# fan1994song/Sentinel

Hardware: AMD Instinct MI355X
Metric: flow-check decisions/sec (node) + % HBM roofline, 10M resources, 1/2/4/8 GPU (higher is better)
Workload: dtype int64; 1 GPU; config3: 10M resources Zipf(1.1), 60% QPS / 10% THREAD / 15% WarmUp / 15% RateLimiter, acquireCount 1 (90%) or 2-5, RT~Exp(20ms) exits; events_per_batch_per_gpu=134217728, entries_per_batch_per_gpu=122837294, parallelism=resource-sharded x1, trace=config-3 batch, seed 3

## Files before the change

### sentinel_amd/csrc/sf_engine.cpp

```cpp
#include <functional>

#include "sf_host.h"

static thread_local std::string g_err;

int fail(int code, const std::string& msg) {
    g_err = msg;
    return code;
}

extern "C" {

int sf_abi_version(void) { return SF_ABI_VERSION; }
const char* sf_last_error(void) { return g_err.c_str(); }

void sf_config_default(sf_config* c) {
    std::memset(c, 0, sizeof *c);
    c->sample_count = 2; c->interval_ms = 1000; c->occupy_timeout_ms = 500; c->cold_factor = 3;
    c->statistic_max_rt = 5000; c->max_resources = 1024; c->max_batch = 1u << 20;
    c->param_capacity = 1u << 16; c->shard_count = 1; c->shard_index = 0; c->device = 0;
    c->cluster_sample_count = 10; c->cluster_interval_ms = 1000; c->exceed_count = 1.0;
    c->max_occupy_ratio = 1.0; c->max_flow_ids = 1024; c->aux_capacity = 65536;
}

static int slot_create(Slot& sl) {
    for (auto& x : sl.evs) HIP_TRY(hipEventCreate(&x));
    for (hipEvent_t* x : {&sl.sorted, &sl.done, &sl.end, &sl.core})
        HIP_TRY(hipEventCreateWithFlags(x, hipEventDisableTiming));
    return SF_OK;
}

void sf_destroy(sf_engine* e) {
    if (!e) return;
    for (hipStream_t x : {e->sstream, e->stream, e->h2d, e->d2h}) if (x) hipStreamSynchronize(x);
    for (Slot& sl : e->slot) { sl.wpool.clear(); sl.pkpool.clear(); }
    for (DevPool* p : {&e->pool, &e->user_dev, &e->user_host, &e->tok.tw.pool, &e->rls.ws.pool, &e->cc.ws.pool, &e->dg.ws.pool, &e->rep.ml_pool})
        p->clear();
    if (e->comm) ncclCommDestroy(e->comm);
    for (Slot& sl : e->slot) {
        const PkStage& p = sl.pk;
        for (hipEvent_t x : {p.h2d, p.d2h, p.consumed, sl.sorted, sl.done, sl.end, sl.core}) if (x) hipEventDestroy(x);
        for (hipEvent_t x : sl.evs) if (x) hipEventDestroy(x);
    }
    for (auto& x : e->rep.ml_ev) if (x) hipEventDestroy(x);
    if (e->ev_en) hipEventDestroy(e->ev_en);
    for (hipStream_t x : {e->h2d, e->d2h, e->stream, e->stream2, e->stream3, e->stream4, e->sstream}) if (x) hipStreamDestroy(x);
    if (e->enstream && e->en_own) hipStreamDestroy(e->enstream);
    delete e;
}

static int work_fill(sf_engine* e, Work& w, DevPool& m) {
    const sf_config& c = e->cfg;
    const size_t N = c.max_batch, R = e->R;
    SF_TRY(m.alloc(&w.keys_in, nz(N * 4))); SF_TRY(m.alloc(&w.keys_out, nz(N * 4))); SF_TRY(m.alloc(&w.perm, nz(N * 4)));
    SF_TRY(m.alloc(&w.pv_in, nz(N * sizeof(PackedEvO)))); SF_TRY(m.alloc(&w.pv_out, nz(N * sizeof(PackedEvO))));
    SF_TRY(m.alloc(&w.err, nz(4)));
    SF_TRY(m.alloc(&w.head_scan, nz(N * 4)));
    SF_TRY(m.alloc(&w.seg_start, nz((N + 1) * 4))); SF_TRY(m.alloc(&w.seg_res, nz(N * 4))); SF_TRY(m.alloc(&w.n_seg, nz(4)));
    SF_TRY(m.alloc(&w.s_meta, nz(N * 4)));
    SF_TRY(m.alloc(&w.s_eref, nz(N * 8))); SF_TRY(m.alloc(&w.s_cts, nz(N * 8)));
    SF_TRY(m.alloc(&w.s_nargs, nz(N))); SF_TRY(m.alloc(&w.s_atag, nz(N * SF_MAX_ARGS))); SF_TRY(m.alloc(&w.s_abits, nz(N * SF_MAX_ARGS * 8)));
    SF_TRY(m.alloc(&w.v_status, nz(N))); SF_TRY(m.alloc(&w.v_wait, nz(N * 4))); SF_TRY(m.alloc(&w.v_rule, nz(N * 2)));
    {
        hipError_t he = query_temp_bytes((uint32_t)N, &w.sort_tmp_bytes, &w.scan_tmp_bytes, &w.pscan_tmp_bytes);
        if (he != hipSuccess) return fail(SF_ERR_DEVICE, "scan temp size query");
    }
    SF_TRY(m.alloc(&w.sort_tmp, nz(w.sort_tmp_bytes)));
    SF_TRY(m.alloc(&w.scan_tmp, nz(w.scan_tmp_bytes)));
    SF_TRY(m.alloc(&w.pscan_tmp, nz(w.pscan_tmp_bytes)));
    w.heavy_min = c.heavy_min_events ? c.heavy_min_events : 512;
    {
        int dev = 0, ncu = 0;
        if (hipGetDevice(&dev) != hipSuccess ||
            hipDeviceGetAttribute(&ncu, hipDeviceAttributeMultiprocessorCount, dev) != hipSuccess) ncu = 256;
        w.stream_grid = 2u * (uint32_t)(ncu > 0 ? ncu : 256);
        w.fill_grid = 8u * (uint32_t)(ncu > 0 ? ncu : 256);
    }
    const size_t SC = std::min<size_t>(N, R) + 1;
    w.seg_cap = (uint32_t)SC;
    SF_TRY(m.alloc(&w.segflag, nz(SC * 4))); SF_TRY(m.alloc(&w.seg_mode, nz(SC))); SF_TRY(m.alloc(&w.lcounts, nz(2 * LCLS * 4)));
    {
        size_t off = 0;
        for (int k = 0; k < LCLS; k++) {
            const size_t lo_len = k == 0 ? 1 : (k == 1 ? 2 : ((size_t)1 << (k - 1)) + 1);
            const size_t cap = lo_len > w.heavy_min ? 0 : std::min<size_t>(SC, N / lo_len + 1);
            w.loff[k] = (uint32_t)off;
            w.lcap[k] = (uint32_t)cap;
            off += cap;
        }
        SF_TRY(m.alloc(&w.light_list, nz(off * 4)));
// ... 6 lines not shown
    SF_TRY(m.alloc(&w.acc_hw, nz((size_t)w.acc_cap * ACC_BYTES))); SF_TRY(m.alloc(&w.acc_sec, nz((size_t)w.acc_cap * ACC_BYTES)));
    SF_TRY(m.alloc(&w.acc_hw_base, nz(SC * 4))); SF_TRY(m.alloc(&w.acc_sec_base, nz(SC * 4))); SF_TRY(m.alloc(&w.seg_hw0, nz(SC * 8)));
    SF_TRY(m.alloc(&w.seg_sec0, nz(SC * 8))); SF_TRY(m.alloc(&w.seg_nhw, nz(SC * 4))); SF_TRY(m.alloc(&w.seg_nsec, nz(SC * 4)));
    SF_TRY(m.alloc(&w.hticks, nz((N / (w.heavy_min + 1) + 2) * 8)));
    SF_TRY(m.alloc(&w.sticks, nz((N / (w.heavy_min + 1) + 2) * 8)));
    SF_TRY(m.alloc(&w.stream_list, nz(SC * 4)));
    SF_TRY(m.alloc(&w.xw_list, nz((N / XW_MIN + 1) * 4)));
    SF_TRY(m.alloc(&w.passbits, nz((N / 64 + 2) * 8)));
    SF_TRY(m.alloc(&w.exit_of, nz(N * 4)));
    SF_TRY(m.alloc(&w.lxfar, nz((N / 64 + 2) * 8)));
    SF_TRY(m.alloc(&w.thr_rec, nz(N * 8)));
    SF_TRY(m.alloc(&w.tile_rc, nz((size_t)w.fill_tile_cap * 4))); SF_TRY(m.alloc(&w.seg_rb, nz(SC * 4))); SF_TRY(m.alloc(&w.seg_re, nz(SC * 4)));
    SF_TRY(m.alloc(&w.vs_cursor, nz(VS_CURSORS(N) * 4)));
    SF_TRY(m.alloc(&w.s_origin, nz(N * 4))); SF_TRY(m.alloc(&w.s_oslot, nz(N * 4))); SF_TRY(m.alloc(&w.ox_cnt, nz(8 * 4)));
    SF_TRY(m.alloc(&w.ox_bflags, nz((N / OX_TILE + 1) * 4))); SF_TRY(m.alloc(&w.ox_bseg, nz((N / OX_TILE + 1) * 8)));
    return SF_OK;
}

static int alloc_work(sf_engine* e, Slot& sl) {
    const int rc = work_fill(e, sl.w, sl.wpool);
    if (rc) { sl.wpool.clear(); sl.w = Work{}; sl.aflags = nullptr; return rc; }
    sl.ready = true;
    return SF_OK;
}

static int create(sf_engine* e);
int sf_create(const sf_config* cfg, sf_engine** out) {
    if (!cfg || !out) return fail(SF_ERR_INVALID, "null argument");
    *out = nullptr;
    const sf_config& c = *cfg;
    if (c.sample_count <= 0 || c.sample_count > SF_MAX_SAMPLE_COUNT || c.interval_ms <= 0 ||
        c.interval_ms % c.sample_count != 0)
        return fail(SF_ERR_INVALID, "sample_count/interval_ms invalid (LeapArray.java:70-87)");
    if (c.max_resources == 0 || c.max_batch == 0) return fail(SF_ERR_INVALID, "max_resources/max_batch must be > 0");
    if (c.shard_count == 0 || c.shard_index >= c.shard_count) return fail(SF_ERR_INVALID, "bad shard");
    int ndev = 0;
    if (hipGetDeviceCount(&ndev) != hipSuccess || ndev <= 0)
        return fail(SF_ERR_DEVICE, "no HIP device visible: the engine has no CPU fallback");
    if (c.device < 0 || c.device >= ndev) return fail(SF_ERR_DEVICE, "device ordinal out of range");
    HIP_TRY(hipSetDevice(c.device));
    hipDeviceProp_t prop;
    HIP_TRY(hipGetDeviceProperties(&prop, c.device));
    if (std::strncmp(prop.gcnArchName, "gfx950", 6) != 0)
        return fail(SF_ERR_DEVICE, std::string("engine is built for gfx950, device is ") + prop.gcnArchName);

    sf_engine* e = new sf_engine();
// ... 63 lines not shown
    HIP_TRY(hipMemsetAsync(st.ptab, 0, pcap * sizeof(ParamSlot), e->stream));
    SF_TRY(e->pool.alloc(&st.pins, nz(256 * 16 * sizeof(unsigned int))));
    SF_TRY(e->pool.alloc(&st.xw_stats, nz(4 * sizeof(unsigned long long))));
    HIP_TRY(hipMemset(e->st.xw_stats, 0, 4 * sizeof(unsigned long long)));
    HIP_TRY(hipMemsetAsync(st.pins, 0, 256 * 16 * sizeof(unsigned int), e->stream));
    HIP_TRY(hipMemsetAsync(st.err, 0, sizeof(int32_t), e->stream));
    HIP_TRY(launch_init_state(st, e->stream));
    e->tok.ts.err = st.err;
    e->tok.ts.exceed_count = c.exceed_count;
    e->tok.ts.shard_count = c.shard_count; e->tok.ts.shard_index = c.shard_index;
    e->tok.ts.max_occupy_ratio = c.max_occupy_ratio;
    SF_TRY(e->pool.alloc(&e->tok.d_sum, nz(sizeof(int64_t))));
    SF_TRY(e->pool.alloc(&st.last_fetch, nz(R * sizeof(int64_t))));
    SF_TRY(e->pool.alloc(&st.last_ts, nz(sizeof(int64_t))));
    {
        const int64_t t_min = INT64_MIN;
        HIP_TRY(hipMemcpyAsync(st.last_ts, &t_min, 8, hipMemcpyHostToDevice, e->stream));
    }
    HIP_TRY(hipMemsetAsync(st.last_fetch, 0xff, R * sizeof(int64_t), e->stream));
    SF_TRY(e->pool.alloc(&e->en, nz(sizeof(EntryNode))));
    SF_TRY(e->pool.alloc(&e->en_acc, nz(sizeof(EntryAcc))));
    HIP_TRY(launch_entry_init(e->en, st.max_rt, e->stream));

    SF_TRY(alloc_work(e, e->slot[0]));
    HIP_TRY(hipStreamSynchronize(e->stream));
    return SF_OK;
}

extern "C++" int local_of(const sf_engine* e, uint32_t res, uint32_t* l) {
    if (res % e->cfg.shard_count != e->cfg.shard_index) return 0;
    *l = res / e->cfg.shard_count;
    return *l < e->R;
}

static void acc_timing(sf_engine* e, Slot& sl) {
    if (!sl.timed) return;
    sl.timed = false;
    hipEvent_t* ev = sl.evs;
    float a = 0, b2 = 0, c = 0, d = 0;
    hipEventElapsedTime(&a, ev[0], ev[1]);
    hipEventElapsedTime(&b2, ev[1], ev[2]);
    hipEventElapsedTime(&c, ev[2], ev[3]);
    hipEventElapsedTime(&d, ev[3], ev[4]);
    float cl = 0, li = 0, hd = 0, hf = 0, hs = 0;
    hipEventElapsedTime(&cl, ev[10], ev[2]);
    hipEventElapsedTime(&li, ev[5], ev[9]);
    if (e->st.n_window_rules) {
        float lq = 0;
        hipEventElapsedTime(&lq, ev[5], ev[16]);
        li = std::max(li, lq);
    }
    hipEventElapsedTime(&hd, ev[5], ev[7]);
    hipEventElapsedTime(&hf, ev[7], ev[8]);
    hipEventElapsedTime(&hs, ev[11], ev[12]);
    e->stats.classify_ms += cl; e->stats.light_ms += li;
    e->stats.heavy_decide_ms += hd; e->stats.heavy_fill_ms += hf; e->stats.stream_ms += hs;
    e->stats.sort_ms += a + b2;
    e->stats.decide_ms += c;
    e->stats.scatter_ms += d;
    e->stats.total_ms += a + b2 + c + d;
}

static int batch_error(int err) {
// ... 578 lines not shown
    e->stats.n_launches++;
}

static int finish_sync(sf_engine* e, Slot& sl, const StagePlan& vout, uint32_t n, bool plain) {
    hipStream_t s = e->stream;
    HIP_TRY(hipEventRecord(sl.core, s));
    HIP_TRY(hipEventRecord(sl.done, s));
    HIP_TRY(hipEventRecord(sl.end, s));
    slot_enqueued(e, sl, n);
    sl.timed = plain && e->timing;
    SF_TRY(vout.download(d2h_on(s)));
    int32_t err = 0;
    uint32_t nseg = 0;
    HIP_TRY(hipMemcpyAsync(&err, sl.w.err, 4, hipMemcpyDeviceToHost, s));
    if (plain) HIP_TRY(hipMemcpyAsync(&nseg, sl.w.n_seg, 4, hipMemcpyDeviceToHost, s));
    HIP_TRY(hipStreamSynchronize(s));
    if (plain) {
        e->stats.n_segments = nseg;
        acc_timing(e, sl);
    }
    return batch_error(err);
}

static int decide_view(sf_engine* e, Slot& sl, DevState& stl, const DevBatch& b, const DevVerdicts& dv,
                       uint32_t p, uint32_t q, bool with_ox, DevBatch& v, DevVerdicts& dvv) {
    hipStream_t s = e->stream;
    Work& w = sl.w;
    v = b;
    v.n = q - p; v.base = p;
    v.res = b.res + p; v.ts = b.ts + p; v.cnt = b.cnt + p; v.flags = b.flags + p;
    v.eref = b.eref ? b.eref + p : nullptr; v.cts = b.cts ? b.cts + p : nullptr;
    v.nargs = b.nargs ? b.nargs + p : nullptr;
    v.atag = b.atag ? b.atag + p : nullptr; v.abits = b.abits ? b.abits + p : nullptr;
    v.origin = b.origin ? b.origin + p : nullptr; v.ctx = b.ctx ? b.ctx + p : nullptr;
    v.sys = e->sys_mask + p; v.vprev = dv.status + p;
    dvv = DevVerdicts{dv.status + p, dv.wait ? dv.wait + p : nullptr, dv.rule ? dv.rule + p : nullptr};
    hipError_t le = launch_sort(stl, w, v, e->cfg.shard_count, e->cfg.shard_index, e->key_bits, s, sl.evs, false);
    OxPlan plan{};
    if (le == hipSuccess && with_ox) {
        SF_TRY(prepare_origins(e, sl, v, s, &plan));
        stl.xtab = e->st.xtab; stl.xcap_mask = e->st.xcap_mask; stl.ax_cap = e->st.ax_cap;
    }
    if (le == hipSuccess)
        le = launch_decide(stl, w, v, dvv, s, e->serial ? s : e->stream2, e->serial ? s : e->stream3,
                           e->serial ? s : e->stream4, sl.evs, false, with_ox ? &plan : nullptr);
    if (le == hipSuccess && with_ox) w.ox_dirty = false;
    if (le != hipSuccess) return fail(SF_ERR_DEVICE, std::string("launch: ") + hipGetErrorString(le));
    return SF_OK;
}

using PreSort = std::function<hipError_t(hipStream_t, int32_t*)>;
struct PackedHook { PreSort pre; bool acsr; uint32_t n_arg_events; };

static int submit_sys_rounds(sf_engine* e, Slot& sl, const DevBatch& staged, const DevVerdicts& dv, const StagePlan& vout,
                             bool with_ox, const PreSort* pre) {
    DevBatch b = staged;
    const uint32_t n = b.n;
    hipStream_t s = e->stream, ss = e->serial ? e->stream : e->sstream;
    Work& w = sl.w;
    SF_TRY(sys_buffers_ensure(e));
// ... 25 lines not shown
        SF_TRY(decide_view(e, sl, stl, b, dv, p, q, with_ox, v, dvv));
        if (qi[1]) le = sys_plan_fix(stl, b, dv, e->sys_mask, e->sys, p, q, e->sys_plan, e->sys_pa, e->sys_pb, s);
        if (le == hipSuccess) le = launch_entry_node(stl, v, dvv.status, e->en, e->en_acc, s);
        if (le != hipSuccess) return fail(SF_ERR_DEVICE, std::string("launch: ") + hipGetErrorString(le));
        p = q;
        rounds++;
    }
    e->stats.sys_rounds += rounds;
    return finish_sync(e, sl, vout, n, false);
}

static int submit_core(sf_engine* e, const sf_event_batch* in, sf_verdicts* out, bool async,
                       const uint8_t* forced = nullptr, const PackedHook* hook = nullptr) {
    if (!e || !in || !out || !out->status) return fail(SF_ERR_INVALID, "null argument");
    if (in->n == 0) return SF_OK;
    SF_TRY(check_event_batch(e, in));
    if (e->sys.check && e->cfg.shard_count > 1 && !forced)
        return fail(SF_ERR_UNSUPPORTED, "SystemRules on a sharded engine: use sf_system_plan + sf_submit_forced "
                                        "+ sf_entry_node_add (the node-wide round protocol)");
    const uint32_t n = in->n;
    hipStream_t s = e->stream, ss = e->serial ? e->stream : e->sstream;
    const bool with_ox = in->origin || e->st.xmap;
    async = async && in->mem != SF_MEM_HOST && out->mem != SF_MEM_HOST && !e->sys.check && !forced;
    if (!async || (with_ox && !e->st.xtab)) SF_TRY(drain(e));
    SF_TRY(reserve_for_batch(e, in, with_ox, hook ? hook->n_arg_events : in->n));
    const PreSort* pre = hook ? &hook->pre : nullptr;
    for (Slot& x : e->slot) {
        if (!async || x.ready) continue;
        HIP_TRY(hipStreamSynchronize(s));
        SF_TRY(alloc_work(e, x));
    }
    Slot& sl = e->slot[e->cur];
    SF_TRY(take_slot(e, sl));
    Work& w = sl.w;
    DevBatch b{};
    DevVerdicts dv{};
    StagePlan vout(false, out->mem == SF_MEM_HOST);
    SF_TRY(stage_batch(e, in, out, ss, b, dv, vout));
    b.acsr = hook && hook->acsr;
    if (forced) {
        SF_TRY(sys_buffers_ensure(e));
        HIP_TRY(hipMemcpyAsync(e->sys_mask, forced, n, hipMemcpyHostToDevice, ss));
        b.sys = e->sys_mask;
    }
    if (e->sys.check && !forced) return submit_sys_rounds(e, sl, b, dv, vout, with_ox, pre);
    if (sl.used) HIP_TRY(hipStreamWaitEvent(ss, e->auth.of && b.origin ? sl.end : sl.done, 0));
    HIP_TRY(hipMemsetAsync(w.err, 0, sizeof(int32_t), ss));
    if (pre) {
        const hipError_t pe = (*pre)(ss, w.err);
        if (pe != hipSuccess) return fail(SF_ERR_DEVICE, std::string("pre-sort: ") + hipGetErrorString(pe));
    }
    SF_TRY(auth_apply(e, sl, b, ss));
    DevState stl = e->st;
    stl.err = w.err;
    hipError_t le = launch_sort(stl, w, b, e->cfg.shard_count, e->cfg.shard_index, e->key_bits, ss, sl.evs, e->timing);
    if (le != hipSuccess) return fail(SF_ERR_DEVICE, std::string("launch: ") + hipGetErrorString(le));
    OxPlan plan{};
    if (with_ox) {
        SF_TRY(prepare_origins(e, sl, b, ss, &plan));
        stl.xtab = e->st.xtab; stl.xcap_mask = e->st.xcap_mask; stl.ax_cap = e->st.ax_cap;
    }
    HIP_TRY(hipEventRecord(sl.sorted, ss));
    HIP_TRY(hipStreamWaitEvent(s, sl.sorted, 0));
    const bool side = async && !e->serial && e->side_mode != 0;
    le = launch_decide(stl, w, b, dv, s, e->serial ? s : e->stream2, e->serial ? s : e->stream3,
                       e->serial ? s : e->stream4, sl.evs, e->timing,
                       with_ox ? &plan : nullptr, false, side ? e->enstream : nullptr);
    if (le != hipSuccess) return fail(SF_ERR_DEVICE, std::string("launch: ") + hipGetErrorString(le));
    if (with_ox) w.ox_dirty = false;
    if (!side && !forced) {
        SF_TRY(en_fence(e));
        le = launch_entry_node(stl, b, dv.status, e->en, e->en_acc, s);
        if (le != hipSuccess) return fail(SF_ERR_DEVICE, std::string("entry node: ") + hipGetErrorString(le));
    }
    if (!async) return finish_sync(e, sl, vout, n, true);
    hipStream_t es = side ? e->enstream : s;
    HIP_TRY(hipEventRecord(sl.core, es));
    HIP_TRY(hipEventRecord(sl.done, es));
// ... 931 lines not shown
```

### sentinel_amd/csrc/sf_host.h

```cpp
#pragma once
#include <hip/hip_runtime.h>

#include <algorithm>
#include <cmath>
#include <cstring>
#include <mutex>
#include <string>
#include <vector>

#include "sf_decide.h"
#include "sf_pkargs.h"
#include "sf_xflow.h"
#include "sf_sysx.h"
#include "sf_token.h"
#include "sf_concur.h"
#include "sf_wire.h"
#include "sf_rls.h"
#include "sf_degrade.h"
#include "sf_mem.h"
#include "sf_worksets.h"
#include <rccl/rccl.h>

using namespace sf;

// ... 115 lines not shown
    hipEvent_t h2d = nullptr, d2h = nullptr;
    hipEvent_t consumed = nullptr;
    bool d2h_pending = false, consumed_pending = false;
    const uint8_t* out_status = nullptr;
    int32_t* err_host = nullptr;
    bool sparse = false;
    sf_sparse_verdicts sp{};
    uint32_t* sp_counts = nullptr;
    const unsigned long long* sp_wl = nullptr; const unsigned long long* sp_rl = nullptr;
};

constexpr int SF_SLOTS = 2;
struct Slot {
    Work w{};
    DevPool wpool{HIP_MEM};
    bool ready = false;
    bool used = false;
    bool timed = false;
    hipEvent_t sorted = nullptr;
    hipEvent_t done = nullptr;
    hipEvent_t end = nullptr;
    hipEvent_t core = nullptr;
    hipEvent_t evs[SF_NUM_EVENTS]{};
    PkStage pk;
    DevPool pkpool{HIP_MEM};
    uint8_t* aflags = nullptr;
};

struct sf_engine {
    sf_config cfg{};
    DevPool pool{HIP_MEM};
    DevPool user_dev{HIP_MEM}, user_host{HIP_MEM};
    hipStream_t stream = nullptr, stream2 = nullptr, stream3 = nullptr, stream4 = nullptr;
    hipStream_t sstream = nullptr;
    hipStream_t enstream = nullptr;
    bool en_own = false;
    int side_mode = 3;
    hipEvent_t ev_en = nullptr;
    bool en_async = false;
    bool serial = false;
    uint32_t R = 0, key_bits = 1;
    DevState st{};
    Slot slot[SF_SLOTS];
    int cur = 0, last = 0;
    unsigned pending = 0;
    SysRule sys{};
    SysPlanDev* sys_plan = nullptr; SysExitQ* sys_pa = nullptr; SysEntQ* sys_pb = nullptr;
    uint8_t* sys_ibuf = nullptr;
    uint8_t* sys_mask = nullptr;
    std::vector<uint32_t> flow_pos;
    uint32_t n_flow = 0, n_prule = 0;
    AuthTables auth{};
    uint64_t p_used = 0, p_pending = 0, p_kmax = 0, p_grows = 0;
    GrowBuf stage_in, stage_out;
    StageBuf plan_sb, en_sb;
    bool timing = false;
    sf_stats stats{};
    std::mutex mu;
    TokHost tok;
    CcHost cc;
    RlsHost rls;
    DgHost dg;
    ReportHost rep;
    SxHost sx;
    EntryNode* en = nullptr;
    EntryAcc* en_acc = nullptr;
// ... 15 lines not shown
```

### sentinel_amd/csrc/sf_internal.h

```cpp
#pragma once
#include <hip/hip_runtime.h>
#include <stdint.h>

#include "../../include/sentinel_flow.h"
#include "sf_degrade.h"
#include "sf_authority.h"

namespace sf {

constexpr int64_t WS_NONE = -(1LL << 62);
constexpr int MINUTE = SF_MINUTE_BUCKETS;
constexpr int MAX_RULES = SF_MAX_RULES_PER_RESOURCE;

struct Bucket {
    int64_t ws, pass, block, exc, succ, rt, occ, min_rt;
};
struct Borrow {
    int64_t ws, pass;
};

enum : int32_t { CT_DEFAULT = 0, CT_WARM_UP = 1, CT_RATE_LIMITER = 2, CT_WARM_UP_RATE_LIMITER = 3 };

struct DevRule {
    uint8_t kind, grade;
// ... 109 lines not shown
struct alignas(8) PackedEv { uint32_t idx, meta; };
struct PackedEvO { uint32_t idx, meta, origin; };
constexpr uint32_t PV_DTS_FAR = 0xffffu;

constexpr int LCLS = 16;
#ifndef SF_SHORT_MAX
#define SF_SHORT_MAX 8
#endif
constexpr uint32_t SHORT_MAX = SF_SHORT_MAX;
__host__ __device__ inline int light_class(uint32_t len) {
    if (len <= 1) return 0;
    const int c = 32 - __builtin_clz(len - 1);
    return c < LCLS - 1 ? c : LCLS - 1;
}
#ifndef SF_FILL_TILE
#define SF_FILL_TILE 2048
#endif
constexpr uint32_t FILL_TILE = SF_FILL_TILE;

struct Work {
    uint32_t n;
    uint32_t* keys_in;   uint32_t* keys_out;
    uint32_t* perm;
    PackedEv* pv_in; PackedEv* pv_out;
    int32_t* err;
    bool ox_dirty;
    uint32_t* head;      uint32_t* head_scan;
    uint32_t* seg_start; uint32_t* seg_res; uint32_t* n_seg;
    uint32_t* s_meta;
    int64_t* s_eref; int64_t* s_cts;
    uint8_t* s_nargs; uint8_t* s_atag; uint64_t* s_abits;
    uint8_t* v_status; int32_t* v_wait; uint16_t* v_rule;
    void* sort_tmp; size_t sort_tmp_bytes;
    void* scan_tmp; size_t scan_tmp_bytes;
    uint32_t seg_cap;
    uint32_t* segflag; uint8_t* seg_mode;
    uint32_t* light_list; uint32_t* heavy_list; uint32_t* counters;
    uint32_t* lcounts;
    uint32_t loff[LCLS];
    uint32_t lcap[LCLS];
    int64_t* pcg; void* pscan_tmp; size_t pscan_tmp_bytes;
    void* segs_lb;
    uint2* fill_tiles; uint32_t fill_tile_cap;
    uint32_t* fill_ntiles;
    uint32_t fill_grid;
    void* acc_hw; void* acc_sec; uint32_t acc_cap;
    uint32_t* acc_hw_base; uint32_t* acc_sec_base; int64_t* seg_hw0; int64_t* seg_sec0;
    uint32_t* seg_nhw; uint32_t* seg_nsec;
    uint32_t heavy_min;
    uint32_t stream_grid;
    uint64_t* hticks;
    uint32_t* stream_list;
    uint32_t* xw_list;
    uint64_t* sticks;
    unsigned long long* passbits;
    uint32_t* exit_of;
// ... 5 lines not shown
    uint32_t* s_origin;
    uint32_t* s_oslot;
    uint32_t* ox_cnt;
    uint32_t* ox_bflags;
    uint2* ox_bseg;
    uint4* ox_pairs; uint32_t ox_pairs_cap;
    uint32_t* ox_plist;
    uint32_t* ox_hmap; size_t ox_hmap_n;
    uint32_t* ox_hslot; size_t ox_hslot_n;
    int64_t* ox_thr;
    void* ox_acc; size_t ox_acc_n;
};
constexpr uint32_t OX_TILE = 2048, OX_LIGHT = 512;
enum : int { OXC_HEAVY = 0, OXC_PAIRS = 1, OXC_PLIST = 2, OXC_OVERFLOW = 3, OXC_RESERVED = 4 };
struct OxAcc {
    unsigned long long pass, block, succ, rt, exc, n_touch, min_rt_key;
};
#ifndef SF_VS_REG
#define SF_VS_REG 14
#endif
constexpr uint32_t VS_REG = SF_VS_REG;
inline size_t VS_CURSORS(size_t N) { return 256 + (N >> VS_REG) + 1024 + 16; }

struct DevBatch {
    uint32_t n;
    const uint32_t* res; const int64_t* ts; const int32_t* cnt; const uint8_t* flags;
    const int64_t* eref; const int64_t* cts;
    uint32_t arg_slots; const uint8_t* nargs; const uint8_t* atag; const uint64_t* abits;
    uint32_t arg_stride;
    const uint32_t* aoff; const uint8_t* etag; const uint64_t* ebits;
    uint32_t acsr;
    const uint32_t* origin; const uint32_t* ctx;
    int64_t base;
    const uint8_t* sys;
    const uint8_t* vprev;
    uint8_t marked;
};
struct DevVerdicts { uint8_t* status; int32_t* wait; uint16_t* rule; };

constexpr uint8_t EVF_SYSBLK = 0x80u;
constexpr uint8_t EVF_SYSREASON_SHIFT = 4;
constexpr uint8_t SYS_NONE = 0xFFu;
constexpr uint8_t SYS_INERT = 0xFEu;
constexpr uint8_t SYSR_OTHER = 7;
constexpr uint8_t SYSR_AUTH = 6;
constexpr int64_t EREF_DEAD = -2;

hipError_t query_temp_bytes(uint32_t max_n, size_t* sort_bytes, size_t* scan_bytes, size_t* pscan_bytes);
hipError_t launch_init_state(const DevState& st, hipStream_t s);
hipError_t launch_rdesc(const DevState& st, hipStream_t s);
hipError_t launch_entry_node(const DevState& st, const DevBatch& b, const uint8_t* vstatus, EntryNode* en,
                             EntryAcc* acc, hipStream_t s);
hipError_t launch_entry_init(EntryNode* en, int64_t max_rt, hipStream_t s);
hipError_t rocprim_scan_bytes(uint32_t n, size_t* bytes);
hipError_t launch_en_pack_ws(const EntryNode* en, int S, int64_t* ws, hipStream_t s);
hipError_t launch_en_pack_vals(const EntryNode* en, int S, const int64_t* gws, int64_t* vals, int64_t* minrt,
                               hipStream_t s);
hipError_t launch_snapshot(const DevState& st, int64_t now, uint32_t shard_count, uint32_t shard_index,
                           uint32_t* counts, uint32_t* offsets, sf_metric_row* out, uint32_t cap, uint32_t* total,
                           void* scan_tmp, size_t scan_bytes, hipStream_t s);
hipError_t mlog_temp_bytes(uint32_t nodes, uint32_t rows, size_t* bytes);
hipError_t launch_mlog_count(const DevState& st, EntryNode* en, bool with_entry, uint32_t shard_count,
                             uint32_t shard_index, int64_t now, unsigned long long* mask, uint32_t* counts,
                             uint32_t* offsets, uint32_t* total, void* tmp, size_t tmp_bytes, unsigned grid,
                             hipEvent_t after_count, hipStream_t s);
hipError_t launch_mlog_rows(const DevState& st, EntryNode* en, bool with_entry, uint32_t shard_count,
                            uint32_t shard_index, int64_t now, const unsigned long long* mask, const uint32_t* offsets,
                            uint32_t n_rows, sf_metric_row* rows, uint8_t* keys, uint8_t* keys_out, uint32_t* order,
                            uint32_t* order_out, void* tmp, size_t tmp_bytes, unsigned grid, hipStream_t s);
hipError_t launch_fmt_len(const sf_metric_row* rows, const uint32_t* order, uint32_t n, const char* names,
                          const uint64_t* name_off, const int32_t* types, uint32_t n_names, int64_t tz,
                          uint64_t* line_len, uint64_t* line_off, uint64_t* total, void* tmp, size_t tmp_bytes,
                          hipStream_t s);
hipError_t launch_fmt_write(const sf_metric_row* rows, const uint32_t* order, uint32_t n, const char* names,
                            const uint64_t* name_off, const int32_t* types, uint32_t n_names, int64_t tz,
                            const uint64_t* line_off, char* out, hipStream_t s);
hipError_t launch_param_stats(const DevState& st, unsigned long long* out, hipStream_t s);
size_t segs_lb_bytes(uint32_t max_n);
hipError_t launch_node_digests(const DevState& st, uint32_t n, unsigned long long* out, hipStream_t s);
hipError_t launch_param_thread_read(const DevState& st, uint32_t l, int idx, uint32_t tag, uint64_t bits,
                                    long long* out, hipStream_t s);
hipError_t launch_sort(const DevState& st, Work& w, const DevBatch& b, uint32_t shard_count, uint32_t shard_index,
                       uint32_t key_bits, hipStream_t s, hipEvent_t* ev, bool timing, bool classify = true);
struct OxWin { int64_t w0s, w0m; uint32_t ws, wm; };
struct OxPlan { uint32_t n_heavy, n_pairs; OxWin win; };
hipError_t launch_decide(const DevState& st, Work& w, const DevBatch& b, const DevVerdicts& out,
                         hipStream_t s, hipStream_t s2, hipStream_t s3, hipStream_t s4, hipEvent_t* ev, bool timing,
                         const OxPlan* ox = nullptr, bool classify = false, hipStream_t sv = nullptr);
hipError_t launch_pk_expand(const uint64_t* ev, const uint32_t* ev4, const uint32_t* ms_end, uint32_t n_ms,
                            const int64_t* xref, const int64_t* xcts, const int32_t* cext,
                            int64_t base, uint32_t n, uint32_t n_exit, uint32_t n_cext, uint2* tile_cnt,
                            uint32_t* res, int64_t* ts, int32_t* cnt, uint8_t* flags, int64_t* eref, int64_t* cts,
                            int32_t* err, hipStream_t s);
struct PkArgIn; struct PkArgOut;
struct PkCopy {
    const uint8_t* etag; const uint64_t* ebits; uint8_t* etag_out; uint64_t* ebits_out;
    const uint32_t* ctx; uint32_t* ctx_out; const uint32_t* origin; uint32_t* origin_out;
};
hipError_t launch_pk_args(const PkArgIn& in, const PkArgOut& out, const PkCopy& cp, int32_t* err, hipStream_t s);
hipError_t launch_sparse_verdicts(const int32_t* wait, const uint16_t* rule, uint32_t n, unsigned long long* wl,
                                  unsigned long long* rl, uint32_t* counts, hipStream_t s);
hipError_t launch_auth_mark(const AuthTables& t, const uint32_t* res, const uint32_t* origin, const uint8_t* flags,
                            uint32_t n, uint8_t mark, uint8_t* out, hipStream_t s);
hipError_t launch_ox_index(const DevState& st, Work& w, const DevBatch& b, uint32_t lim, hipStream_t s);
hipError_t launch_ox_apply(const DevState& st, Work& w, const DevBatch& b, uint32_t n_heavy, uint32_t n_pairs,
                           const OxWin& win, hipStream_t s);
// ... 8 lines not shown
```

### sentinel_amd/csrc/sf_kernels.hip

```cpp
#include <cstring>
#include <rocprim/rocprim.hpp>

#include "sf_pkargs.h"
#include "sf_rsort.h"
#include "sf_stream.h"
#include "sf_system.h"
#include "sf_xflow.h"

namespace sf {

__global__ void k_init_state(DevState st, size_t n_sec, size_t n_min) {
    size_t i = (size_t)blockIdx.x * blockDim.x + threadIdx.x;
    size_t stride = (size_t)gridDim.x * blockDim.x;
    for (size_t k = i; k < n_sec; k += stride) {
        st.second[k] = fresh_bucket(WS_NONE, st.max_rt);
        st.borrow[k].ws = WS_NONE; st.borrow[k].pass = 0;
    }
    for (size_t k = i; k < n_min; k += stride) st.minute[k] = fresh_bucket(WS_NONE, st.max_rt);
    for (size_t k = i; k < st.R; k += stride) st.threads[k] = 0;
}

__global__ void k_segs(DevBatch b, SortedEv ev, const uint8_t* s_atag,
                       const uint32_t* keys, const uint32_t* head_scan, uint32_t* seg_start, uint32_t* seg_res,
                       uint32_t* n_seg, uint32_t* segflag, int64_t* last_ts, const int32_t* err, bool exit_marks,
// ... 1774 lines not shown
    const uint4 w = make_uint4(v, v, v, v);
    for (size_t i = t; i < body; i += stride) q[i] = w;
}
static void launch_fill(const FillSet& f, hipStream_t s) {
    if (!f.k) return;
    size_t most = 0;
    for (int r = 0; r < f.k; r++) most = std::max(most, f.n[r] / 16 + 16);
    hipLaunchKernelGGL(k_fill, dim3((unsigned)std::min<size_t>(2048, (most + 255) / 256), (unsigned)f.k), dim3(256), 0, s, f);
}

using PcIter = rocprim::transform_iterator<rocprim::counting_iterator<uint32_t>, EntryCount, int64_t>;
using HeadIter = rocprim::transform_iterator<rocprim::counting_iterator<uint32_t>, HeadFlag, uint32_t>;
#ifndef SF_HEAD_SCAN_CFG
#define SF_HEAD_SCAN_CFG rocprim::scan_config<256, 21, rocprim::block_load_method::block_load_transpose, \
    rocprim::block_store_method::block_store_transpose, rocprim::block_scan_algorithm::using_warp_scan>
#endif
#ifndef SF_PC_SCAN_CFG
#define SF_PC_SCAN_CFG rocprim::scan_config<256, 12, rocprim::block_load_method::block_load_transpose, \
    rocprim::block_store_method::block_store_transpose, rocprim::block_scan_algorithm::using_warp_scan>
#endif
using HeadScanCfg = SF_HEAD_SCAN_CFG;
using PcScanCfg = SF_PC_SCAN_CFG;

hipError_t query_temp_bytes(uint32_t max_n, size_t* sort_bytes, size_t* scan_bytes, size_t* pscan_bytes) {
    *sort_bytes = rs_scratch_bytes();
    hipError_t e;
    HeadIter hit(rocprim::counting_iterator<uint32_t>(0), HeadFlag{nullptr});
    e = rocprim::inclusive_scan<HeadScanCfg>(nullptr, *scan_bytes, hit, (uint32_t*)nullptr, (size_t)max_n,
                                rocprim::plus<uint32_t>());
    if (e != hipSuccess) return e;
    PcIter it(rocprim::counting_iterator<uint32_t>(0), EntryCount{SortedEv{}});
    return rocprim::inclusive_scan<PcScanCfg>(nullptr, *pscan_bytes, it, (int64_t*)nullptr, (size_t)max_n,
                                   rocprim::plus<int64_t>());
}

hipError_t rocprim_scan_bytes(uint32_t n, size_t* bytes) {
    return rocprim::exclusive_scan(nullptr, *bytes, (uint32_t*)nullptr, (uint32_t*)nullptr, 0u, (size_t)n,
                                   rocprim::plus<uint32_t>());
}

__global__ void k_rdesc(DevState st, RDesc* out) {
    const uint32_t r = blockIdx.x * blockDim.x + threadIdx.x;
    if (r < st.R) out[r] = make_rdesc(st, r);
}
hipError_t launch_rdesc(const DevState& st, hipStream_t s) {
    hipLaunchKernelGGL(k_rdesc, dim3(blocks(st.R, 256)), dim3(256), 0, s, st, (RDesc*)st.rdesc);
    return hipGetLastError();
}
// ... 6 lines not shown

static void launch_classify(const DevState& st, Work& w, const DevBatch& b, hipStream_t s, hipEvent_t* ev, bool timing) {
    const uint32_t n = b.n;
    FillSet f;
    f.add(w.counters, 16 * sizeof(uint32_t), 0);
    f.add(w.lcounts, 2 * LCLS * sizeof(uint32_t), 0);
    f.add(w.passbits, ((size_t)n / 64 + 2) * 8, 0);
    if (st.n_stream_rules) f.add(w.lxfar, ((size_t)n / 64 + 2) * 8, 0);
    launch_fill(f, s);
    const uint32_t max_seg = n < st.R ? n : st.R;
    if (timing) hipEventRecord(ev[10], s);
    hipLaunchKernelGGL(k_classify, dim3(blocks(max_seg, 1024)), dim3(1024), 0, s, st, w, sorted_ev(w, b));
    HeavyCtx hc = heavy_ctx(w);
    StreamCtx sc{w.stream_list, w.counters + 5, w.seg_cap, nullptr, w.counters + 7};
    hipLaunchKernelGGL(k_fill_tiles, dim3(2), dim3(1024), 0, s, hc, sc, w.fill_tiles, w.fill_tile_cap, w.fill_ntiles);
    if (timing) hipEventRecord(ev[2], s);
}

static bool segs_one_pass() {
    static const bool v = [] { const char* x = getenv("SF_SEGS_LB"); return !(x && x[0] == '0'); }();
    return v;
}

hipError_t launch_sort(const DevState& st, Work& w, const DevBatch& b, uint32_t shard_count, uint32_t shard_index,
                       uint32_t key_bits, hipStream_t s, hipEvent_t* ev, bool timing, bool classify) {
    const uint32_t n = b.n;
    if (n == 0) return hipSuccess;
    const unsigned T = 256;
    if (timing) hipEventRecord(ev[0], s);
    hipError_t e;
    const bool org = b.origin != nullptr;
    const RsBatchSrc src{b, shard_count, shard_index, st.R, st.err, st.last_ts, st.xmap};
    if (org) {
        const RsSinkFinal<PackedEvO> fin{b, w.keys_out, w.perm, w.s_meta, w.s_origin, w.s_nargs, w.s_atag, w.s_abits};
        e = rs_sort(src, n, key_bits, w.keys_in, (PackedEvO*)w.pv_in, w.head_scan, (PackedEvO*)w.pv_out, fin,
                    w.sort_tmp, s);
    } else {
        const RsSinkFinal<PackedEv> fin{b, w.keys_out, w.perm, w.s_meta, nullptr, w.s_nargs, w.s_atag, w.s_abits};
        e = rs_sort(src, n, key_bits, w.keys_in, w.pv_in, w.head_scan, w.pv_out, fin, w.sort_tmp, s);
    }
    if (e != hipSuccess) return e;
    if (!segs_one_pass()) {
        HeadIter hit(rocprim::counting_iterator<uint32_t>(0), HeadFlag{w.keys_out});
        e = rocprim::inclusive_scan<HeadScanCfg>(w.scan_tmp, w.scan_tmp_bytes, hit, w.head_scan, (size_t)n,
                                    rocprim::plus<uint32_t>(), s);
        if (e != hipSuccess) return e;
    }
    hipMemsetAsync(w.segflag, 0, (size_t)(n < st.R ? n : st.R) * 4, s);
    if (timing) hipEventRecord(ev[1], s);
    if (!segs_one_pass()) {
        hipLaunchKernelGGL(k_segs, dim3(blocks(n, T)), dim3(T), 0, s, b, sorted_ev(w, b), w.s_atag, w.keys_out,
                           w.head_scan, w.seg_start, w.seg_res, w.n_seg, w.segflag, st.last_ts, st.err,
                           st.n_prule != 0, st.prio_seen);
    } else {
        if (st.n_window_rules) launch_segs3<true>(st, w, b, s);
        else launch_segs3<false>(st, w, b, s);
    }
    if (classify) launch_classify(st, w, b, s, ev, timing);
    return hipGetLastError();
}

#ifndef SF_VS_T
// ... 516 lines not shown
```

### sentinel_amd/csrc/sf_rsort.h

```cpp
#pragma once
#include "sf_decide.h"

namespace sf {

#ifndef SF_RS_DB
#define SF_RS_DB 8
#endif
#ifndef SF_RS_W
#define SF_RS_W 8
#endif
constexpr int RS_DB = SF_RS_DB, RS_NB = 1 << RS_DB, RS_W = SF_RS_W;
constexpr int RS_T = RS_W * 64;
constexpr uint32_t RS_MAX_CHUNKS = 1024;

__device__ __forceinline__ uint32_t rs_meta(const DevBatch& b, uint32_t i, int64_t ts, int64_t ts0) {
    const uint8_t f = b.flags[i];
    const uint8_t sr = (b.sys && (f & SF_EV_IN) && !(f & SF_EV_EXIT)) ? b.sys[i] : SYS_NONE;
    return ev_pack(ts, ts0, f, sr, b.cnt[i], b.marked != 0);
}

__device__ __forceinline__ void rs_put_origin(uint32_t*, uint32_t, const PackedEv&) {}
__device__ __forceinline__ void rs_cp(PackedEv& d, const PackedEv& s) { d.idx = s.idx; d.meta = s.meta; }
__device__ __forceinline__ void rs_cp(PackedEvO& d, const PackedEvO& s) { d.idx = s.idx; d.meta = s.meta; d.origin = s.origin; }
__device__ __forceinline__ void rs_put_origin(uint32_t* o, uint32_t j, const PackedEvO& v) { o[j] = v.origin; }
// ... 270 lines not shown
inline void rs_chunks(uint32_t n, uint32_t* C, uint32_t* chunk) {
    constexpr uint32_t TILE = RsGeom<V>::TILE;
    uint32_t c = (n + TILE - 1) / TILE;
    if (c > RS_MAX_CHUNKS) c = RS_MAX_CHUNKS;
    uint32_t ch = (n + c - 1) / c;
    ch = (ch + TILE - 1) / TILE * TILE;
    *chunk = ch;
    *C = (n + ch - 1) / ch;
}

template <class SRC, class SINK, class V>
inline void rs_launch_pass(const SRC& src, const SINK& sink, uint32_t n, uint32_t shift, uint32_t mask, void* scratch,
                           hipStream_t s) {
    uint32_t C, chunk;
    rs_chunks<V>(n, &C, &chunk);
    uint32_t* h = (uint32_t*)scratch;
    uint32_t* tot = h + (size_t)RS_MAX_CHUNKS * RS_NB;
    hipLaunchKernelGGL(k_rs_count<SRC>, dim3(C), dim3(256), 0, s, src, n, chunk, shift, mask, h);
    hipLaunchKernelGGL(k_rs_scan, dim3(RS_NB), dim3(RS_MAX_CHUNKS), 0, s, h, C, tot);
    hipLaunchKernelGGL((k_rs_pass<SRC, SINK, V>), dim3(C), dim3(RS_T), 0, s, src, sink, n, chunk, shift, mask,
                       (const uint32_t*)h, (const uint32_t*)tot);
}

template <class V>
hipError_t rs_sort(const RsBatchSrc& src, uint32_t n, uint32_t key_bits, uint32_t* keys_a, V* pv_a, uint32_t* keys_b,
                   V* pv_b, const RsSinkFinal<V>& fin, void* scratch, hipStream_t s) {
    if (n == 0) return hipSuccess;
    const uint32_t kb = key_bits ? key_bits : 1;
    const uint32_t P = (kb + RS_DB - 1) / RS_DB;
    const uint32_t D = (kb + P - 1) / P;
    const uint32_t mask = (1u << D) - 1u;
    const RsSinkKV<V> sa{keys_a, pv_a}, sb{keys_b, pv_b};
    for (uint32_t p = 0; p < P; p++) {
        const uint32_t shift = p * D;
        const bool last = p + 1 == P;
        const RsSinkKV<V>& mid = (p & 1) ? sb : sa;
        if (p == 0) {
            if (last) rs_launch_pass<RsBatchSrc, RsSinkFinal<V>, V>(src, fin, n, shift, mask, scratch, s);
            else rs_launch_pass<RsBatchSrc, RsSinkKV<V>, V>(src, mid, n, shift, mask, scratch, s);
        } else {
            const RsSinkKV<V>& prev = (p & 1) ? sa : sb;
            const RsArraySrc<V> as{prev.k, prev.v};
            if (last) rs_launch_pass<RsArraySrc<V>, RsSinkFinal<V>, V>(as, fin, n, shift, mask, scratch, s);
            else rs_launch_pass<RsArraySrc<V>, RsSinkKV<V>, V>(as, mid, n, shift, mask, scratch, s);
        }
    }
    return hipGetLastError();
}

}
```

Measured before the change: 9.980 billion decisions/s.

## Split radix sort so early passes run before slot acquisition

Splits the radix sort into early passes, which write into an engine-wide sort scratch, and a final pass that writes the per-slot outputs. In async mode the early passes are launched on the staging stream before waiting for the slot to free, so they can overlap the previous batch's decide work. Errors from the early passes are folded into the slot's error word by a small kernel. The per-slot sort buffers are removed, but the single shared scratch adds a cross-batch hazard unless stream ordering keeps it safe. The new path is on by default and can be turned off with SF_EARLY_SORT.

```diff
diff --git a/sentinel_amd/csrc/sf_engine.cpp b/sentinel_amd/csrc/sf_engine.cpp
--- a/sentinel_amd/csrc/sf_engine.cpp
+++ b/sentinel_amd/csrc/sf_engine.cpp
@@ -25,6 +25,7 @@
 
 static int slot_create(Slot& sl) {
     for (auto& x : sl.evs) HIP_TRY(hipEventCreate(&x));
+    for (auto& x : sl.early) HIP_TRY(hipEventCreate(&x));
     for (hipEvent_t* x : {&sl.sorted, &sl.done, &sl.end, &sl.core})
         HIP_TRY(hipEventCreateWithFlags(x, hipEventDisableTiming));
     return SF_OK;
@@ -34,6 +35,7 @@
     if (!e) return;
     for (hipStream_t x : {e->sstream, e->stream, e->h2d, e->d2h}) if (x) hipStreamSynchronize(x);
     for (Slot& sl : e->slot) { sl.wpool.clear(); sl.pkpool.clear(); }
+    e->scpool.clear();
     for (DevPool* p : {&e->pool, &e->user_dev, &e->user_host, &e->tok.tw.pool, &e->rls.ws.pool, &e->cc.ws.pool, &e->dg.ws.pool, &e->rep.ml_pool})
         p->clear();
     if (e->comm) ncclCommDestroy(e->comm);
@@ -41,6 +43,7 @@
         const PkStage& p = sl.pk;
         for (hipEvent_t x : {p.h2d, p.d2h, p.consumed, sl.sorted, sl.done, sl.end, sl.core}) if (x) hipEventDestroy(x);
         for (hipEvent_t x : sl.evs) if (x) hipEventDestroy(x);
+        for (hipEvent_t x : sl.early) if (x) hipEventDestroy(x);
     }
     for (auto& x : e->rep.ml_ev) if (x) hipEventDestroy(x);
     if (e->ev_en) hipEventDestroy(e->ev_en);
@@ -53,7 +56,7 @@
     const sf_config& c = e->cfg;
     const size_t N = c.max_batch, R = e->R;
     SF_TRY(m.alloc(&w.keys_in, nz(N * 4))); SF_TRY(m.alloc(&w.keys_out, nz(N * 4))); SF_TRY(m.alloc(&w.perm, nz(N * 4)));
-    SF_TRY(m.alloc(&w.pv_in, nz(N * sizeof(PackedEvO)))); SF_TRY(m.alloc(&w.pv_out, nz(N * sizeof(PackedEvO))));
+    SF_TRY(m.alloc(&w.pv_in, nz(N * sizeof(PackedEvO))));
     SF_TRY(m.alloc(&w.err, nz(4)));
     SF_TRY(m.alloc(&w.head_scan, nz(N * 4)));
     SF_TRY(m.alloc(&w.seg_start, nz((N + 1) * 4))); SF_TRY(m.alloc(&w.seg_res, nz(N * 4))); SF_TRY(m.alloc(&w.n_seg, nz(4)));
@@ -62,10 +65,9 @@
     SF_TRY(m.alloc(&w.s_nargs, nz(N))); SF_TRY(m.alloc(&w.s_atag, nz(N * SF_MAX_ARGS))); SF_TRY(m.alloc(&w.s_abits, nz(N * SF_MAX_ARGS * 8)));
     SF_TRY(m.alloc(&w.v_status, nz(N))); SF_TRY(m.alloc(&w.v_wait, nz(N * 4))); SF_TRY(m.alloc(&w.v_rule, nz(N * 2)));
     {
-        hipError_t he = query_temp_bytes((uint32_t)N, &w.sort_tmp_bytes, &w.scan_tmp_bytes, &w.pscan_tmp_bytes);
+        hipError_t he = query_temp_bytes((uint32_t)N, &w.scan_tmp_bytes, &w.pscan_tmp_bytes);
         if (he != hipSuccess) return fail(SF_ERR_DEVICE, "scan temp size query");
     }
-    SF_TRY(m.alloc(&w.sort_tmp, nz(w.sort_tmp_bytes)));
     SF_TRY(m.alloc(&w.scan_tmp, nz(w.scan_tmp_bytes)));
     SF_TRY(m.alloc(&w.pscan_tmp, nz(w.pscan_tmp_bytes)));
     w.heavy_min = c.heavy_min_events ? c.heavy_min_events : 512;
@@ -118,6 +120,23 @@
     if (rc) { sl.wpool.clear(); sl.w = Work{}; sl.aflags = nullptr; return rc; }
     sl.ready = true;
     return SF_OK;
+}
+
+static int alloc_sort_scratch(sf_engine* e) {
+    const size_t N = e->cfg.max_batch;
+    SortScratch& sc = e->sc;
+    DevPool& m = e->scpool;
+    const auto fill = [&]() -> int {
+        for (int k = 0; k < 2; k++) {
+            SF_TRY(m.alloc(&sc.keys[k], nz(N * 4)));
+            SF_TRY(m.alloc(&sc.pv[k], nz(N * sizeof(PackedEvO))));
+        }
+        SF_TRY(m.alloc(&sc.hist, nz(sort_hist_bytes())));
+        return m.alloc(&sc.err, nz(sizeof(int32_t)));
+    };
+    const int rc = fill();
+    if (rc) { m.clear(); sc = SortScratch{}; }
+    return rc;
 }
 
 static int create(sf_engine* e);
@@ -227,7 +246,9 @@
     SF_TRY(e->pool.alloc(&e->en_acc, nz(sizeof(EntryAcc))));
     HIP_TRY(launch_entry_init(e->en, st.max_rt, e->stream));
 
+    if (const char* v = getenv("SF_EARLY_SORT")) e->early_sort = v[0] != '0';
     SF_TRY(alloc_work(e, e->slot[0]));
+    SF_TRY(alloc_sort_scratch(e));
     HIP_TRY(hipStreamSynchronize(e->stream));
     return SF_OK;
 }
@@ -243,7 +264,7 @@
     sl.timed = false;
     hipEvent_t* ev = sl.evs;
     float a = 0, b2 = 0, c = 0, d = 0;
-    hipEventElapsedTime(&a, ev[0], ev[1]);
+    hipEventElapsedTime(&a, sl.t0, ev[1]);
     hipEventElapsedTime(&b2, ev[1], ev[2]);
     hipEventElapsedTime(&c, ev[2], ev[3]);
     hipEventElapsedTime(&d, ev[3], ev[4]);
@@ -868,6 +889,16 @@
     return batch_error(err);
 }
 
+static hipError_t sort_whole(sf_engine* e, Slot& sl, const DevState& stl, const DevBatch& b, hipStream_t s, bool timing) {
+    const sf_config& c = e->cfg;
+    sl.t0 = sl.evs[0];
+    hipError_t le = launch_sort_early(stl, e->sc, b, c.shard_count, c.shard_index, e->key_bits, stl.err, s,
+                                      timing ? sl.t0 : nullptr);
+    if (le == hipSuccess)
+        le = launch_sort_last(stl, e->sc, sl.w, b, c.shard_count, c.shard_index, e->key_bits, s, sl.evs, timing);
+    return le;
+}
+
 static int decide_view(sf_engine* e, Slot& sl, DevState& stl, const DevBatch& b, const DevVerdicts& dv,
                        uint32_t p, uint32_t q, bool with_ox, DevBatch& v, DevVerdicts& dvv) {
     hipStream_t s = e->stream;
@@ -881,7 +912,7 @@
     v.origin = b.origin ? b.origin + p : nullptr; v.ctx = b.ctx ? b.ctx + p : nullptr;
     v.sys = e->sys_mask + p; v.vprev = dv.status + p;
     dvv = DevVerdicts{dv.status + p, dv.wait ? dv.wait + p : nullptr, dv.rule ? dv.rule + p : nullptr};
-    hipError_t le = launch_sort(stl, w, v, e->cfg.shard_count, e->cfg.shard_index, e->key_bits, s, sl.evs, false);
+    hipError_t le = sort_whole(e, sl, stl, v, s, false);
     OxPlan plan{};
     if (le == hipSuccess && with_ox) {
         SF_TRY(prepare_origins(e, sl, v, s, &plan));
@@ -953,7 +984,8 @@
     hipStream_t s = e->stream, ss = e->serial ? e->stream : e->sstream;
     const bool with_ox = in->origin || e->st.xmap;
     async = async && in->mem != SF_MEM_HOST && out->mem != SF_MEM_HOST && !e->sys.check && !forced;
-    if (!async || (with_ox && !e->st.xtab)) SF_TRY(drain(e));
+    const bool drained_ox = with_ox && !e->st.xtab;
+    if (!async || drained_ox) SF_TRY(drain(e));
     SF_TRY(reserve_for_batch(e, in, with_ox, hook ? hook->n_arg_events : in->n));
     const PreSort* pre = hook ? &hook->pre : nullptr;
     for (Slot& x : e->slot) {
@@ -962,12 +994,23 @@
         SF_TRY(alloc_work(e, x));
     }
     Slot& sl = e->slot[e->cur];
-    SF_TRY(take_slot(e, sl));
     Work& w = sl.w;
     DevBatch b{};
     DevVerdicts dv{};
     StagePlan vout(false, out->mem == SF_MEM_HOST);
-    SF_TRY(stage_batch(e, in, out, ss, b, dv, vout));
+    const bool early = e->early_sort && async && !e->serial && !hook && !drained_ox && !(e->auth.of && in->origin) &&
+                       sort_passes(e->key_bits) > 1;
+    hipEvent_t t0 = nullptr;
+    if (early) {
+        SF_TRY(stage_batch(e, in, out, ss, b, dv, vout));
+        t0 = sl.early[sl.t0 == sl.early[0]];
+        HIP_TRY(hipMemsetAsync(e->sc.err, 0, sizeof(int32_t), ss));
+        const hipError_t ee = launch_sort_early(e->st, e->sc, b, e->cfg.shard_count, e->cfg.shard_index, e->key_bits,
+                                                e->sc.err, ss, e->timing ? t0 : nullptr);
+        if (ee != hipSuccess) return fail(SF_ERR_DEVICE, std::string("launch: ") + hipGetErrorString(ee));
+    }
+    SF_TRY(take_slot(e, sl));
+    if (!early) SF_TRY(stage_batch(e, in, out, ss, b, dv, vout));
     b.acsr = hook && hook->acsr;
     if (forced) {
         SF_TRY(sys_buffers_ensure(e));
@@ -977,6 +1020,7 @@
     if (e->sys.check && !forced) return submit_sys_rounds(e, sl, b, dv, vout, with_ox, pre);
     if (sl.used) HIP_TRY(hipStreamWaitEvent(ss, e->auth.of && b.origin ? sl.end : sl.done, 0));
     HIP_TRY(hipMemsetAsync(w.err, 0, sizeof(int32_t), ss));
+    if (early) HIP_TRY(launch_err_fold(e->sc.err, w.err, ss));
     if (pre) {
         const hipError_t pe = (*pre)(ss, w.err);
         if (pe != hipSuccess) return fail(SF_ERR_DEVICE, std::string("pre-sort: ") + hipGetErrorString(pe));
@@ -984,7 +1028,11 @@
     SF_TRY(auth_apply(e, sl, b, ss));
     DevState stl = e->st;
     stl.err = w.err;
-    hipError_t le = launch_sort(stl, w, b, e->cfg.shard_count, e->cfg.shard_index, e->key_bits, ss, sl.evs, e->timing);
+    hipError_t le;
+    if (early) {
+        sl.t0 = t0;
+        le = launch_sort_last(stl, e->sc, w, b, e->cfg.shard_count, e->cfg.shard_index, e->key_bits, ss, sl.evs, e->timing);
+    } else le = sort_whole(e, sl, stl, b, ss, e->timing);
     if (le != hipSuccess) return fail(SF_ERR_DEVICE, std::string("launch: ") + hipGetErrorString(le));
     OxPlan plan{};
     if (with_ox) {
diff --git a/sentinel_amd/csrc/sf_host.h b/sentinel_amd/csrc/sf_host.h
--- a/sentinel_amd/csrc/sf_host.h
+++ b/sentinel_amd/csrc/sf_host.h
@@ -161,6 +161,8 @@
     hipEvent_t end = nullptr;
     hipEvent_t core = nullptr;
     hipEvent_t evs[SF_NUM_EVENTS]{};
+    hipEvent_t early[2]{};
+    hipEvent_t t0 = nullptr;
     PkStage pk;
     DevPool pkpool{HIP_MEM};
     uint8_t* aflags = nullptr;
@@ -181,6 +183,9 @@
     uint32_t R = 0, key_bits = 1;
     DevState st{};
     Slot slot[SF_SLOTS];
+    SortScratch sc{};
+    DevPool scpool{HIP_MEM};
+    bool early_sort = true;
     int cur = 0, last = 0;
     unsigned pending = 0;
     SysRule sys{};
diff --git a/sentinel_amd/csrc/sf_internal.h b/sentinel_amd/csrc/sf_internal.h
--- a/sentinel_amd/csrc/sf_internal.h
+++ b/sentinel_amd/csrc/sf_internal.h
@@ -155,7 +155,7 @@
     uint32_t n;
     uint32_t* keys_in;   uint32_t* keys_out;
     uint32_t* perm;
-    PackedEv* pv_in; PackedEv* pv_out;
+    PackedEv* pv_in;
     int32_t* err;
     bool ox_dirty;
     uint32_t* head;      uint32_t* head_scan;
@@ -164,7 +164,6 @@
     int64_t* s_eref; int64_t* s_cts;
     uint8_t* s_nargs; uint8_t* s_atag; uint64_t* s_abits;
     uint8_t* v_status; int32_t* v_wait; uint16_t* v_rule;
-    void* sort_tmp; size_t sort_tmp_bytes;
     void* scan_tmp; size_t scan_tmp_bytes;
     uint32_t seg_cap;
     uint32_t* segflag; uint8_t* seg_mode;
@@ -216,6 +215,13 @@
 constexpr uint32_t VS_REG = SF_VS_REG;
 inline size_t VS_CURSORS(size_t N) { return 256 + (N >> VS_REG) + 1024 + 16; }
 
+struct SortScratch {
+    uint32_t* keys[2];
+    PackedEv* pv[2];
+    void* hist;
+    int32_t* err;
+};
+
 struct DevBatch {
     uint32_t n;
     const uint32_t* res; const int64_t* ts; const int32_t* cnt; const uint8_t* flags;
@@ -240,7 +246,9 @@
 constexpr uint8_t SYSR_AUTH = 6;
 constexpr int64_t EREF_DEAD = -2;
 
-hipError_t query_temp_bytes(uint32_t max_n, size_t* sort_bytes, size_t* scan_bytes, size_t* pscan_bytes);
+hipError_t query_temp_bytes(uint32_t max_n, size_t* scan_bytes, size_t* pscan_bytes);
+size_t sort_hist_bytes();
+uint32_t sort_passes(uint32_t key_bits);
 hipError_t launch_init_state(const DevState& st, hipStream_t s);
 hipError_t launch_rdesc(const DevState& st, hipStream_t s);
 hipError_t launch_entry_node(const DevState& st, const DevBatch& b, const uint8_t* vstatus, EntryNode* en,
@@ -274,8 +282,12 @@
 hipError_t launch_node_digests(const DevState& st, uint32_t n, unsigned long long* out, hipStream_t s);
 hipError_t launch_param_thread_read(const DevState& st, uint32_t l, int idx, uint32_t tag, uint64_t bits,
                                     long long* out, hipStream_t s);
-hipError_t launch_sort(const DevState& st, Work& w, const DevBatch& b, uint32_t shard_count, uint32_t shard_index,
-                       uint32_t key_bits, hipStream_t s, hipEvent_t* ev, bool timing, bool classify = true);
+hipError_t launch_sort_early(const DevState& st, const SortScratch& sc, const DevBatch& b, uint32_t shard_count,
+                             uint32_t shard_index, uint32_t key_bits, int32_t* err, hipStream_t s, hipEvent_t start);
+hipError_t launch_sort_last(const DevState& st, const SortScratch& sc, Work& w, const DevBatch& b, uint32_t shard_count,
+                            uint32_t shard_index, uint32_t key_bits, hipStream_t s, hipEvent_t* ev, bool timing,
+                            bool classify = true);
+hipError_t launch_err_fold(const int32_t* from, int32_t* to, hipStream_t s);
 struct OxWin { int64_t w0s, w0m; uint32_t ws, wm; };
 struct OxPlan { uint32_t n_heavy, n_pairs; OxWin win; };
 hipError_t launch_decide(const DevState& st, Work& w, const DevBatch& b, const DevVerdicts& out,
diff --git a/sentinel_amd/csrc/sf_kernels.hip b/sentinel_amd/csrc/sf_kernels.hip
--- a/sentinel_amd/csrc/sf_kernels.hip
+++ b/sentinel_amd/csrc/sf_kernels.hip
@@ -1820,8 +1820,10 @@
 using HeadScanCfg = SF_HEAD_SCAN_CFG;
 using PcScanCfg = SF_PC_SCAN_CFG;
 
-hipError_t query_temp_bytes(uint32_t max_n, size_t* sort_bytes, size_t* scan_bytes, size_t* pscan_bytes) {
-    *sort_bytes = rs_scratch_bytes();
+size_t sort_hist_bytes() { return rs_scratch_bytes(); }
+uint32_t sort_passes(uint32_t key_bits) { return rs_plan(key_bits).P; }
+
+hipError_t query_temp_bytes(uint32_t max_n, size_t* scan_bytes, size_t* pscan_bytes) {
     hipError_t e;
     HeadIter hit(rocprim::counting_iterator<uint32_t>(0), HeadFlag{nullptr});
     e = rocprim::inclusive_scan<HeadScanCfg>(nullptr, *scan_bytes, hit, (uint32_t*)nullptr, (size_t)max_n,
@@ -1874,22 +1876,42 @@
     return v;
 }
 
-hipError_t launch_sort(const DevState& st, Work& w, const DevBatch& b, uint32_t shard_count, uint32_t shard_index,
-                       uint32_t key_bits, hipStream_t s, hipEvent_t* ev, bool timing, bool classify) {
+__global__ void k_err_fold(const int32_t* from, int32_t* to) {
+    const int32_t v = *from;
+    if (v) *to = v;
+}
+hipError_t launch_err_fold(const int32_t* from, int32_t* to, hipStream_t s) {
+    hipLaunchKernelGGL(k_err_fold, dim3(1), dim3(1), 0, s, from, to);
+    return hipGetLastError();
+}
+
+hipError_t launch_sort_early(const DevState& st, const SortScratch& sc, const DevBatch& b, uint32_t shard_count,
+                             uint32_t shard_index, uint32_t key_bits, int32_t* err, hipStream_t s, hipEvent_t start) {
+    if (b.n == 0) return hipSuccess;
+    if (start) hipEventRecord(start, s);
+    const RsBatchSrc src{b, shard_count, shard_index, st.R, err, st.last_ts, st.xmap};
+    if (b.origin)
+        return rs_sort_early(src, b.n, key_bits, sc.keys[0], (PackedEvO*)sc.pv[0], sc.keys[1], (PackedEvO*)sc.pv[1],
+                             sc.hist, s);
+    return rs_sort_early(src, b.n, key_bits, sc.keys[0], sc.pv[0], sc.keys[1], sc.pv[1], sc.hist, s);
+}
+
+hipError_t launch_sort_last(const DevState& st, const SortScratch& sc, Work& w, const DevBatch& b, uint32_t shard_count,
+                            uint32_t shard_index, uint32_t key_bits, hipStream_t s, hipEvent_t* ev, bool timing,
+                            bool classify) {
     const uint32_t n = b.n;
     if (n == 0) return hipSuccess;
     const unsigned T = 256;
-    if (timing) hipEventRecord(ev[0], s);
     hipError_t e;
-    const bool org = b.origin != nullptr;
     const RsBatchSrc src{b, shard_count, shard_index, st.R, st.err, st.last_ts, st.xmap};
-    if (org) {
+    if (b.origin) {
         const RsSinkFinal<PackedEvO> fin{b, w.keys_out, w.perm, w.s_meta, w.s_origin, w.s_nargs, w.s_atag, w.s_abits};
-        e = rs_sort(src, n, key_bits, w.keys_in, (PackedEvO*)w.pv_in, w.head_scan, (PackedEvO*)w.pv_out, fin,
-                    w.sort_tmp, s);
+        e = rs_sort_last(src, n, key_bits, sc.keys[0], (const PackedEvO*)sc.pv[0], sc.keys[1], (const PackedEvO*)sc.pv[1],
+                         fin, sc.hist, s);
     } else {
         const RsSinkFinal<PackedEv> fin{b, w.keys_out, w.perm, w.s_meta, nullptr, w.s_nargs, w.s_atag, w.s_abits};
-        e = rs_sort(src, n, key_bits, w.keys_in, w.pv_in, w.head_scan, w.pv_out, fin, w.sort_tmp, s);
+        e = rs_sort_last(src, n, key_bits, sc.keys[0], (const PackedEv*)sc.pv[0], sc.keys[1], (const PackedEv*)sc.pv[1],
+                         fin, sc.hist, s);
     }
     if (e != hipSuccess) return e;
     if (!segs_one_pass()) {
diff --git a/sentinel_amd/csrc/sf_rsort.h b/sentinel_amd/csrc/sf_rsort.h
--- a/sentinel_amd/csrc/sf_rsort.h
+++ b/sentinel_amd/csrc/sf_rsort.h
@@ -316,30 +316,46 @@
                        (const uint32_t*)h, (const uint32_t*)tot);
 }
 
-template <class V>
-hipError_t rs_sort(const RsBatchSrc& src, uint32_t n, uint32_t key_bits, uint32_t* keys_a, V* pv_a, uint32_t* keys_b,
-                   V* pv_b, const RsSinkFinal<V>& fin, void* scratch, hipStream_t s) {
-    if (n == 0) return hipSuccess;
+struct RsPlan { uint32_t P, D, mask; };
+inline RsPlan rs_plan(uint32_t key_bits) {
     const uint32_t kb = key_bits ? key_bits : 1;
     const uint32_t P = (kb + RS_DB - 1) / RS_DB;
     const uint32_t D = (kb + P - 1) / P;
-    const uint32_t mask = (1u << D) - 1u;
+    return RsPlan{P, D, (1u << D) - 1u};
+}
+
+template <class V>
+hipError_t rs_sort_early(const RsBatchSrc& src, uint32_t n, uint32_t key_bits, uint32_t* keys_a, V* pv_a,
+                         uint32_t* keys_b, V* pv_b, void* scratch, hipStream_t s) {
+    const RsPlan pl = rs_plan(key_bits);
+    if (n == 0 || pl.P < 2) return hipSuccess;
     const RsSinkKV<V> sa{keys_a, pv_a}, sb{keys_b, pv_b};
-    for (uint32_t p = 0; p < P; p++) {
-        const uint32_t shift = p * D;
-        const bool last = p + 1 == P;
+    for (uint32_t p = 0; p + 1 < pl.P; p++) {
+        const uint32_t shift = p * pl.D;
         const RsSinkKV<V>& mid = (p & 1) ? sb : sa;
-        if (p == 0) {
-            if (last) rs_launch_pass<RsBatchSrc, RsSinkFinal<V>, V>(src, fin, n, shift, mask, scratch, s);
-            else rs_launch_pass<RsBatchSrc, RsSinkKV<V>, V>(src, mid, n, shift, mask, scratch, s);
-        } else {
+        if (p == 0) rs_launch_pass<RsBatchSrc, RsSinkKV<V>, V>(src, mid, n, shift, pl.mask, scratch, s);
+        else {
             const RsSinkKV<V>& prev = (p & 1) ? sa : sb;
             const RsArraySrc<V> as{prev.k, prev.v};
-            if (last) rs_launch_pass<RsArraySrc<V>, RsSinkFinal<V>, V>(as, fin, n, shift, mask, scratch, s);
-            else rs_launch_pass<RsArraySrc<V>, RsSinkKV<V>, V>(as, mid, n, shift, mask, scratch, s);
+            rs_launch_pass<RsArraySrc<V>, RsSinkKV<V>, V>(as, mid, n, shift, pl.mask, scratch, s);
         }
     }
     return hipGetLastError();
 }
 
-}
+template <class V>
+hipError_t rs_sort_last(const RsBatchSrc& src, uint32_t n, uint32_t key_bits, const uint32_t* keys_a, const V* pv_a,
+                        const uint32_t* keys_b, const V* pv_b, const RsSinkFinal<V>& fin, void* scratch,
+                        hipStream_t s) {
+    if (n == 0) return hipSuccess;
+    const RsPlan pl = rs_plan(key_bits);
+    const uint32_t p = pl.P - 1, shift = p * pl.D;
+    if (p == 0) rs_launch_pass<RsBatchSrc, RsSinkFinal<V>, V>(src, fin, n, shift, pl.mask, scratch, s);
+    else {
+        const RsArraySrc<V> as{(p & 1) ? keys_a : keys_b, (p & 1) ? pv_a : pv_b};
+        rs_launch_pass<RsArraySrc<V>, RsSinkFinal<V>, V>(as, fin, n, shift, pl.mask, scratch, s);
+    }
+    return hipGetLastError();
+}
+
+}
```

New measurement: 9.925 billion decisions/s. About the same (-0.6%).
